# ChanghyeonKim93/nonlinear_optimizer_for_slam

Measured on AMD Instinct MI355X. Metric: ndt6_gauss_newton_residual_blocks_per_sec, higher is better.
Workload: dtype f64

## Files before the change

include/nos.h:

```cpp
#ifndef NOS_H_
#define NOS_H_

#include <stddef.h>
#include <stdint.h>

#ifdef __cplusplus
extern "C" {
#endif

#define NOS_NDT_PLANES 15
#define NOS_REPROJ_PLANES 5
#define NOS_NDT6_OUT 28
#define NOS_NDT3_OUT 10
#define NOS_REPROJ_OUT 28

typedef enum nos_status {
  NOS_OK = 0,
  NOS_ERR_INVALID_ARGUMENT = 1,
  NOS_ERR_NO_DEVICE = 2,
  NOS_ERR_HIP = 3,
  NOS_ERR_OUT_OF_MEMORY = 4,
  NOS_ERR_WRONG_KIND = 5,
  NOS_ERR_UNSUPPORTED = 6
} nos_status;
// ... 215 lines not shown
                            nos_register_report* reports);

int nos_voxel_map_register6_batch(nos_voxel_map* map, nos_scan* const* scans, int32_t n_problems, double* R, double* t,
                                  const nos_loss* loss, const nos_register_options* ropt, const nos_lm_options* options,
                                  nos_register_report* reports);
int nos_voxel_map_register3_batch(nos_voxel_map* map, nos_scan* const* scans, int32_t n_problems, double* R, double* t,
                                  const nos_loss* loss, const nos_register_options* ropt, const nos_lm_options* options,
                                  nos_register_report* reports);

typedef struct nos_pose_score {
  uint64_t matches;
  uint64_t matched_points;
  double cost;
  double reserved;
} nos_pose_score;

int nos_ndt_score_batch(nos_ndt_map* map, nos_scan* const* scans, int32_t n_problems, const double* R ,
                        const double* t , const nos_loss* loss, int max_neighbors, nos_pose_score* scores);
int nos_voxel_map_score_batch(nos_voxel_map* map, nos_scan* const* scans, int32_t n_problems, const double* R ,
                              const double* t , const nos_loss* loss, int max_neighbors, nos_pose_score* scores);

int nos_debug_lm_step(nos_ctx* ctx, int dof, const double* sums, const double settings[4], double state[22]);

int nos_debug_voxel_finish(uint32_t count, const double sums[9], const int64_t cell[3], double voxel_resolution,
                           const double params[3], int flags, double mean[3], double sqrt_information[9], unsigned char* valid);

int nos_debug_voxel_moments(uint32_t count, const double sums[9], const int64_t cell[3], double src_resolution,
                            const double R[9], const double t[3], double dst_resolution,
                            int64_t cell_out[3], double sums_out[9]);

typedef struct nos_pose_graph nos_pose_graph;
int nos_pgo_create(nos_ctx* ctx, size_t n_poses, const double* poses, size_t n_edges,
                   const int32_t* ref, const int32_t* qry, const double* meas,
                   const double* switch_init, const unsigned char* switch_free,
                   const unsigned char* fixed, nos_pose_graph** out_pg);
int nos_pgo_destroy(nos_pose_graph* pg);
size_t nos_pgo_num_unknowns(const nos_pose_graph* pg);
int nos_pgo_linearize(nos_pose_graph* pg, double* cost, double* gradient_norm);
int nos_pgo_solve(nos_pose_graph* pg, double lambda, int max_iterations, double rel_tolerance,
                  int* iterations, double* rel_residual, double* step_norm);
int nos_pgo_retract(nos_pose_graph* pg);
int nos_pgo_get_state(nos_pose_graph* pg, double* poses, double* switches);
int nos_pgo_get_vector(nos_pose_graph* pg, int which, double* out);
int nos_pgo_matvec(nos_pose_graph* pg, double lambda, const double* x, double* y);
int nos_pgo_layout_info(const nos_pose_graph* pg, unsigned long long info[8]);
int nos_pgo_time_sweep(nos_pose_graph* pg, int which, double lambda, int repeats, double* ms_per_sweep);
// ... 28 lines not shown
```

nonlinear_optimizer_for_slam_amd/_lib.py:

```python
import ctypes
import os

_HERE = os.path.dirname(os.path.abspath(__file__))
CSRC = os.path.join(_HERE, "csrc")
LIB_HIP = os.environ.get("NOS_HIP_LIB") or os.path.join(CSRC, "libnos_hip.so")
LIB_HOST = os.path.join(CSRC, "libnos_host.so")

c_double_p = ctypes.POINTER(ctypes.c_double)
c_void_pp = ctypes.POINTER(ctypes.c_void_p)

NOS_OK = 0
NOS_F64 = 0
NOS_F32 = 1
NOS_LOSS_NONE = 0
NOS_LOSS_EXPONENTIAL = 1
NOS_LOSS_HUBER = 2

C_ABI_SYMBOLS = (
    "nos_ctx_create", "nos_ctx_destroy", "nos_ctx_num_devices", "nos_ctx_set_stream",
    "nos_ctx_synchronize", "nos_comm_get_unique_id", "nos_ctx_comm_init", "nos_ctx_comm_size", "nos_ctx_comm_init_shm", "nos_ctx_comm_init_shm_device", "nos_comm_shm_unlink", "nos_ctx_comm_destroy",
    "nos_ctx_comm_allreduce", "nos_ndt_dataset_create", "nos_reproj_dataset_create",
    "nos_ndt_dataset_create_from_device", "nos_reproj_dataset_create_from_device",
    "nos_ndt_dataset_create_from_records", "nos_reproj_dataset_create_from_records",
    "nos_dataset_download", "nos_ndt_map_create", "nos_ndt_map_destroy", "nos_ndt_map_size", "nos_scan_create",
    "nos_scan_destroy", "nos_scan_size", "nos_scan_sort_by_cell", "nos_scan_order", "nos_scan_filter", "nos_scan_points", "nos_ndt_match", "nos_ndt_indexed_dataset_create", "nos_ndt_match_indexed", "nos_indexed_dataset_info", "nos_indexed_dataset_download", "nos_ndt_map_build", "nos_map_stats_size",
    "nos_map_stats_get", "nos_map_stats_get_eigen", "nos_map_stats_destroy",
    "nos_voxel_map_create", "nos_voxel_map_insert", "nos_voxel_map_insert_scan", "nos_voxel_map_info", "nos_voxel_map_snapshot",
    "nos_voxel_map_stats", "nos_voxel_map_match", "nos_voxel_map_match_indexed", "nos_voxel_map_prune", "nos_voxel_map_memory", "nos_voxel_map_merge", "nos_voxel_map_destroy", "nos_dataset_drop_last_matches", "nos_pgo_create", "nos_pgo_destroy", "nos_pgo_num_unknowns",
    "nos_pgo_linearize", "nos_pgo_solve", "nos_pgo_retract", "nos_pgo_get_state", "nos_pgo_get_vector",
    "nos_pgo_matvec", "nos_pgo_time_sweep", "nos_pgo_layout_info", "nos_debug_lm_step", "nos_debug_voxel_finish", "nos_debug_voxel_moments", "nos_dataset_destroy", "nos_dataset_size", "nos_dataset_dtype", "nos_dataset_stream_bytes",
    "nos_dataset_set_simd_class",
    "nos_ndt6_accumulate", "nos_ndt3_accumulate", "nos_reproj_accumulate",
    "nos_ndt6_accumulate_async", "nos_ndt3_accumulate_async", "nos_reproj_accumulate_async",
    "nos_ndt6_solve", "nos_ndt3_solve", "nos_reproj_solve",
    "nos_ndt6_solve_batch", "nos_ndt3_solve_batch", "nos_reproj_solve_batch",
    "nos_ndt6_register_batch", "nos_ndt3_register_batch", "nos_voxel_map_register6_batch", "nos_voxel_map_register3_batch",
    "nos_ndt_score_batch", "nos_voxel_map_score_batch",
    "nos_ctx_set_launch", "nos_ctx_set_option", "nos_ctx_get_option", "nos_runtime_info", "nos_ctx_comm_rccl_count",
    "nos_ctx_last_kernel", "nos_ctx_profile_begin", "nos_ctx_profile_end", "nos_ndt6_time_kernel", "nos_reproj_time_kernel",
    "nos_ndt3_time_kernel", "nos_status_string", "nos_last_error", "nos_version",
)


class NosLoss(ctypes.Structure):
    _fields_ = [("kind", ctypes.c_int32), ("reserved", ctypes.c_int32),
                ("a", ctypes.c_double), ("b", ctypes.c_double)]


class NosLmOptions(ctypes.Structure):
    _fields_ = [("max_iterations", ctypes.c_int32), ("launches_in_flight", ctypes.c_int32),
                ("gradient_tolerance", ctypes.c_double), ("parameter_tolerance", ctypes.c_double),
                ("cost_history", ctypes.POINTER(ctypes.c_double))]

# ... 132 lines not shown
        if hasattr(lib, "nos_voxel_map_match"):
            lib.nos_voxel_map_match.argtypes = [vp, vp, dp, dp, i, i, c_void_pp, ctypes.POINTER(sz)]
        if hasattr(lib, "nos_voxel_map_match_indexed"):
            lib.nos_voxel_map_match_indexed.argtypes = [vp, vp, dp, dp, i, i, i, c_void_pp, ctypes.POINTER(sz)]
            lib.nos_indexed_dataset_info.argtypes = [vp, ctypes.POINTER(i), ctypes.POINTER(sz)]
            lib.nos_indexed_dataset_download.argtypes = [vp, ctypes.POINTER(ctypes.POINTER(ctypes.c_int32)), dp]
    if hasattr(lib, "nos_dataset_drop_last_matches"):
        lib.nos_dataset_drop_last_matches.argtypes = [vp, sz]
    ip = ctypes.POINTER(ctypes.c_int32)
    lib.nos_pgo_create.argtypes = [vp, sz, dp, sz, ip, ip, dp, dp, ctypes.c_char_p, ctypes.c_char_p, c_void_pp]
    lib.nos_pgo_destroy.argtypes = [vp]
    lib.nos_pgo_num_unknowns.argtypes = [vp]
    lib.nos_pgo_num_unknowns.restype = sz
    lib.nos_pgo_linearize.argtypes = [vp, dp, dp]
    lib.nos_pgo_solve.argtypes = [vp, ctypes.c_double, i, ctypes.c_double, ctypes.POINTER(i), dp, dp]
    lib.nos_pgo_retract.argtypes = [vp]
    lib.nos_pgo_get_state.argtypes = [vp, dp, dp]
    lib.nos_pgo_get_vector.argtypes = [vp, i, dp]
    lib.nos_pgo_matvec.argtypes = [vp, ctypes.c_double, dp, dp]
    if hasattr(lib, "nos_pgo_layout_info"):
        lib.nos_pgo_layout_info.argtypes = [vp, ctypes.POINTER(ctypes.c_ulonglong)]
    if hasattr(lib, "nos_debug_lm_step"):
        lib.nos_debug_lm_step.argtypes = [vp, i, dp, dp, dp]
    if hasattr(lib, "nos_debug_voxel_finish"):
        lib.nos_debug_voxel_finish.argtypes = [ctypes.c_uint32, dp, ctypes.POINTER(ctypes.c_int64), ctypes.c_double, dp, i, dp, dp,
                                               ctypes.POINTER(ctypes.c_ubyte)]
    if hasattr(lib, "nos_debug_voxel_moments"):
        i64p = ctypes.POINTER(ctypes.c_int64)
        lib.nos_debug_voxel_moments.argtypes = [ctypes.c_uint32, dp, i64p, ctypes.c_double, dp, dp, ctypes.c_double, i64p, dp]
    if hasattr(lib, "nos_pgo_time_sweep"):
        lib.nos_pgo_time_sweep.argtypes = [vp, i, ctypes.c_double, i, dp]
    lib.nos_dataset_destroy.argtypes = [vp]
    lib.nos_dataset_set_simd_class.argtypes = [vp, ctypes.c_int]
    lib.nos_dataset_set_simd_class.restype = ctypes.c_int
    lib.nos_dataset_size.argtypes = [vp]
    lib.nos_dataset_size.restype = sz
    lib.nos_dataset_dtype.argtypes = [vp]
    lib.nos_dataset_stream_bytes.argtypes = [vp]
    lib.nos_dataset_stream_bytes.restype = sz
    lib.nos_ndt6_accumulate.argtypes = [vp, dp, dp, lp, dp]
    lib.nos_ndt3_accumulate.argtypes = [vp, dp, dp, lp, dp]
    lib.nos_reproj_accumulate.argtypes = [vp, dp, dp, dp, lp, ctypes.c_double, dp]
    lib.nos_ndt6_accumulate_async.argtypes = [vp, dp, dp, lp, vp]
    lib.nos_ndt3_accumulate_async.argtypes = [vp, dp, dp, lp, vp]
    lib.nos_reproj_accumulate_async.argtypes = [vp, dp, dp, dp, lp, ctypes.c_double, vp]
    lmo, lmr = ctypes.POINTER(NosLmOptions), ctypes.POINTER(NosLmReport)
# ... 33 lines not shown
```

nonlinear_optimizer_for_slam_amd/csrc/assemble_one_launch.hpp:

```cpp
#pragma once

#include "assemble_pass.hpp"

namespace nos {

constexpr size_t kSingleBlockMaxElements = size_t(1024) * 15;

template <typename Problem, typename T, int BLOCK, bool NT>
__device__ __forceinline__ int single_block_loop(const TiledLayout& L, typename Problem::Params& P, uint32_t n_chunks,
                                                 LmDevice& s_lm, double* s_sum, double* __restrict__ cost_history,
                                                 int history_capacity) {
  constexpr int kF = Problem::kFields;
  constexpr int kOut = Problem::kOut;
  const T* __restrict__ base = static_cast<const T*>(L.base);
  int executed = 0;
  while (s_lm.st.done == 0) {
    set_pose(P, &s_lm);
    T acc[kOut];
#pragma unroll
    for (int k = 0; k < kOut; ++k) acc[k] = T(0);
    constexpr uint32_t kRound = (kF * sizeof(T) > 64) ? 2 : 4;
    for (uint32_t c = 0; c < n_chunks; c += kRound) {
      T x[kRound][kF][1];
      uint64_t i0[kRound];
// ... 107 lines not shown
__device__ __forceinline__ void state_load_sc1(const LmDevice* lm, nos_host::LmState& st) {
  const double* d = reinterpret_cast<const double*>(&lm->st);
  double* s = reinterpret_cast<double*>(&st);
  constexpr int kWords = int(sizeof(nos_host::LmState) / sizeof(double));
#pragma unroll
  for (int k = 0; k < kWords; ++k) s[k] = sc1_load(d + k);
}

template <int FIELDS, int ELEM>
struct ResidentShape;
template <>
struct ResidentShape<15, 8> { static constexpr int RI = 3, LI = 3; };
template <>
struct ResidentShape<15, 4> { static constexpr int RI = 3, LI = 4; };
template <>
struct ResidentShape<5, 8> { static constexpr int RI = 9, LI = 7; };
template <>
struct ResidentShape<5, 4> { static constexpr int RI = 10, LI = 14; };

template <typename Problem, typename T>
struct StreamRegRounds { static constexpr int kRR = 3; };
template <int LOSS>
struct StreamRegRounds<Ndt6Problem<float, LOSS>, float> { static constexpr int kRR = 0; };
constexpr int kStreamRegRoundsMax = 3;

template <typename Problem, typename T, int BLOCK, int RI, int LI, int SI = 0, bool SPF = false, bool NT = false>
__global__ __launch_bounds__(BLOCK) void solve_cluster_kernel(TiledLayout L, typename Problem::Params P,
                                                             double* __restrict__ partials, LmDevice* lm, ClusterCtl* ctl,
                                                             double* __restrict__ cost_history, int history_capacity,
                                                             double* entry_host, unsigned long long* seq_host,
                                                             unsigned long long seq, uint32_t items_per_lane,
                                                             const Mailbox* mail = nullptr, uint32_t stream_lds = 0u,
                                                             uint32_t stream_reg = 0u) {
  constexpr int kF = Problem::kFields;
  constexpr int kOut = Problem::kOut;
  constexpr int kCols = 32;
  constexpr int kSlices = BLOCK / kCols;
  const T* __restrict__ base = static_cast<const T*>(L.base);
  constexpr int kRF = kF;
  extern __shared__ __align__(16) unsigned char resident_raw[];
  T* resident = reinterpret_cast<T*>(resident_raw);
  __shared__ int s_flag;
  __shared__ int s_fast;
  __shared__ double red[kSlices][kCols];
  __shared__ double s_tot[kLmTotDoubles(kOut)];
  __shared__ double s_lmd_raw[(sizeof(LmDevice) + 7) / 8];
  LmDevice& s_lmd = *reinterpret_cast<LmDevice*>(s_lmd_raw);
// ... 7 lines not shown
  [[maybe_unused]] constexpr int kXccCol = 28;
  [[maybe_unused]] const unsigned int my_xcc = xcc_id();
  const uint64_t block_base = uint64_t(blockIdx.x) * BLOCK * J;
  auto fetch = [&](uint32_t j, T (&dst)[kRF]) -> bool {
    const uint64_t i = block_base + uint64_t(j) * BLOCK + threadIdx.x;
    const bool ok = i < L.n;
    const uint64_t ic = ok ? i : 0;
    const uint64_t off = (ic >> L.tile_shift) * L.tile_stride + (ic & L.tile_mask);
    T xt[kF][1];
#pragma unroll
    for (int f = 0; f < kF; ++f) load_items<T, 1, false>(base + field_offset<Problem>(L, ic, off, f), xt[f]);
#pragma unroll
    for (int f = 0; f < kF; ++f) dst[f] = ok ? xt[f][0] : T(0);
    return ok;
  };
  auto evaluate_resident = [&](const T (&xi)[kRF], bool ok, T (&acc_)[kOut]) { Problem::item(xi, P, ok, acc_); };
  T x[RI > 0 ? RI : 1][kRF];
  bool valid[RI > 0 ? RI : 1];
  static_assert(SI == 0 || (RI == 0 && LI == 0), "the streaming form keeps nothing resident");
  constexpr int kSI = SI > 0 ? SI : 1;
  [[maybe_unused]] T xs[kF][kSI];
  [[maybe_unused]] uint64_t xs_i0 = 0;
  [[maybe_unused]] constexpr int kRR = (SI > 0 && !SPF) ? StreamRegRounds<Problem, T>::kRR : 0;
  static_assert(kRR <= kStreamRegRoundsMax, "the option's range covers every instantiation");
  [[maybe_unused]] T xr[kRR > 0 ? kRR : 1][kF][kSI];
  [[maybe_unused]] const uint32_t my_rounds = blockIdx.x < J ? (J - blockIdx.x + gridDim.x - 1) / gridDim.x : 0u;
  [[maybe_unused]] const uint32_t lds_k = SI > 0 ? min(stream_lds, my_rounds > 0u ? my_rounds - 1u : 0u) : 0u;
  [[maybe_unused]] const uint32_t reg_k = kRR > 0 ? min(min(stream_reg, uint32_t(kRR)), (my_rounds > 0u ? my_rounds - 1u : 0u) - lds_k) : 0u;
  [[maybe_unused]] const uint32_t alt_k = min(lds_k, reg_k);
  [[maybe_unused]] auto chip_round = [&](uint32_t i) -> uint32_t {
    return uint32_t(uint64_t(i + 1u) * my_rounds / (lds_k + reg_k + 1u));
  };
  [[maybe_unused]] auto lds_slot_round = [&](uint32_t sl) -> uint32_t {
    return sl < lds_k ? chip_round(sl < alt_k ? 2u * sl : alt_k + sl) : ~0u;
  };
  [[maybe_unused]] const uint32_t lds_r0 = lds_slot_round(0u);
  [[maybe_unused]] const uint32_t lds_r1 = lds_slot_round(1u);
  [[maybe_unused]] const uint32_t lds_r2 = lds_slot_round(2u);
  [[maybe_unused]] uint32_t reg_r[kRR > 0 ? kRR : 1];
#pragma unroll
  for (int j = 0; j < (kRR > 0 ? kRR : 1); ++j)
    reg_r[j] = uint32_t(j) < reg_k ? chip_round(uint32_t(j) < alt_k ? 2u * uint32_t(j) + 1u : alt_k + uint32_t(j)) : ~0u;
#pragma unroll
  for (int j = 0; j < (kRR > 0 ? kRR : 1); ++j)
#pragma unroll
    for (int f = 0; f < kF; ++f)
#pragma unroll
      for (int e = 0; e < kSI; ++e) xr[j][f][e] = T(0);
  [[maybe_unused]] auto lds_round = [&](uint32_t s) -> uint32_t { return s == 0u ? lds_r0 : s == 1u ? lds_r1 : s == 2u ? lds_r2 : ~0u; };
  [[maybe_unused]] auto fetch_chunk = [&](uint32_t c, T (&dst)[kF][kSI]) -> uint64_t {
    const uint64_t i0 = uint64_t(c) * (uint64_t(BLOCK) * kSI) + uint64_t(threadIdx.x) * kSI;
    const uint64_t off = (i0 >> L.tile_shift) * L.tile_stride + (i0 & L.tile_mask);
#pragma unroll
    for (int f = 0; f < kF; ++f) load_items<T, kSI, NT>(base + field_offset<Problem>(L, i0, off, f), dst[f]);
    return i0;
  };
  if constexpr (SI > 0) {
    if (blockIdx.x < J) xs_i0 = fetch_chunk(blockIdx.x, xs);
  }
#pragma unroll
  for (int j = 0; j < RI; ++j) {
    valid[j] = false;
    if (uint32_t(j) < J) {
      valid[j] = fetch(uint32_t(j), x[j]);
    } else {
#pragma unroll
      for (int f = 0; f < kRF; ++f) x[j][f] = T(0);
    }
  }
  if constexpr (LI > 0) {
    for (uint32_t j = RI; j < J; ++j) {
      T xi[kRF];
      (void)fetch(j, xi);
#pragma unroll
      for (int f = 0; f < kRF; ++f) resident[(size_t(j - RI) * kRF + f) * BLOCK + threadIdx.x] = xi[f];
    }
  }
// ... 159 lines not shown
      }
    } else
    if (sizeof(T) == 8 && J >= uint32_t(RI)) {
#pragma unroll
      for (int j = 0; j < RI; ++j) evaluate_resident(x[j], valid[j], acc);
    } else {
#pragma unroll
      for (int j = 0; j < RI; ++j)
        if (uint32_t(j) < J) evaluate_resident(x[j], valid[j], acc);
    }
    if constexpr (LI > 0) {
      for (uint32_t j = RI; j < J; ++j) {
        T xi[kRF];
#pragma unroll
        for (int f = 0; f < kRF; ++f) xi[f] = resident[(size_t(j - RI) * kRF + f) * BLOCK + threadIdx.x];
        evaluate_resident(xi, (block_base + uint64_t(j) * BLOCK + threadIdx.x) < L.n, acc);
      }
    }
    double dacc[kOut];
#pragma unroll
    for (int k = 0; k < kOut; ++k) dacc[k] = double(acc[k]);
    NOS_RES_STAMP(0)
    {
      TaggedUnit* const block_units = reinterpret_cast<TaggedUnit*>(partials);
      TaggedUnit* const group_units = block_units + size_t(kClusterMaxBlocks) * 32;
      const unsigned long long tag = (seq << 24) | ((unsigned long long)it + 1ull);
      const double mine = block_reduce_value<kOut, BLOCK>(dacc);
      const bool probe = it == 0u && allow_fast;
      if (threadIdx.x < kOut) {
        if (s_fast != 0)
          tagged_store_plain(block_units + size_t(blockIdx.x) * 32 + threadIdx.x, mine, tag);
        else
          tagged_store(block_units + size_t(blockIdx.x) * 32 + threadIdx.x, mine, tag);
      } else if (probe && threadIdx.x == kXccCol) {
        tagged_store(block_units + size_t(blockIdx.x) * 32 + kXccCol, double(my_xcc), tag);
      }
      NOS_RES_STAMP(1)
      const unsigned long long deadline = wall_clock64() + (multi ? kClusterMailboxTimeoutTicks : kClusterTimeoutTicks);
      auto await = [&](const TaggedUnit* u, double* value) -> bool {
        unsigned int polls = 0;
        for (;;) {
          const TaggedUnit got = tagged_load(u);
          if (got.seq == tag) {
            *value = got.value;
            return true;
          }
          if ((++polls & 63u) == 0u &&
              (__hip_atomic_load(&ctl->abort, __ATOMIC_RELAXED, __HIP_MEMORY_SCOPE_AGENT) != 0u || wall_clock64() > deadline)) {
            __hip_atomic_store(&ctl->abort, 1u, __ATOMIC_RELAXED, __HIP_MEMORY_SCOPE_AGENT);
            s_flag = 2;
            return false;
          }
        }
      };
      const int col = threadIdx.x % kCols;
      const int slice = threadIdx.x / kCols;
      if (blockIdx.x < n_groups) {
        const unsigned int g_size = (gridDim.x - blockIdx.x + 7u) >> 3;
        double gsum = 0.0;
        for (unsigned int m0 = 0; m0 < g_size; m0 += kSlices) {
          const unsigned int m = m0 + slice;
          double v = 0.0;
          if (m < g_size && (col < kOut || (probe && col == kXccCol))) {
            (void)await(block_units + size_t(blockIdx.x + 8u * m) * 32 + col, &v);
            if (col == kXccCol) v = v == double(my_xcc) ? 0.0 : 1.0;
          }
          red[slice][col] = v;
          __syncthreads();
          if (threadIdx.x < kOut || (probe && threadIdx.x == kXccCol)) {
#pragma unroll
            for (int sl = 0; sl < kSlices; ++sl) gsum += red[sl][threadIdx.x];
          }
          __syncthreads();
        }
        if ((threadIdx.x < kOut || (probe && threadIdx.x == kXccCol)) && s_flag != 2)
          tagged_store(group_units + (size_t(it & 1u) * 8 + blockIdx.x) * 32 + threadIdx.x, gsum, tag);
      }
      if (!multi || blockIdx.x == 0) {
        double v = 0.0;
        if (slice < int(n_groups) && (col < kOut || (probe && col == kXccCol)) && s_flag != 2)
          (void)await(group_units + (size_t(it & 1u) * 8 + slice) * 32 + col, &v);
        if (slice < 8) red[slice][col] = v;
      }
      __syncthreads();
      if (multi) {
        TaggedUnit* const global_units = group_units + size_t(2) * 8 * 32;
        if (blockIdx.x == 0) {
          if (threadIdx.x < kCols && s_flag != 2) {
            double tot = 0.0;
            if (threadIdx.x < kOut || (probe && threadIdx.x == kXccCol))
              for (unsigned int g = 0; g < n_groups; ++g) tot += red[g][threadIdx.x];
            s_local[threadIdx.x] = tot;
          }
          __syncthreads();
          if (threadIdx.x < kWave) {
            const Mailbox mb = *mail;
            const unsigned long long round = s_round0 + (unsigned long long)it + 1ull;
            const unsigned int xtag = (unsigned int)(round % 0xFFFFFFFFull) + 1u;
            const size_t parity = size_t(round & 1ull);
            const size_t units_base = size_t(mb.n_ranks) * 2 * kMailSlotDoubles;
            const int lane = int(threadIdx.x);
            const bool giving_up = s_flag == 2;
            unsigned long long* const own = reinterpret_cast<unsigned long long*>(mb.peers[mb.rank] + units_base);
            if (giving_up) {
              if (lane < mb.n_ranks)
                __hip_atomic_store(reinterpret_cast<unsigned long long*>(mb.peers[lane] + units_base) +
                                       (size_t(mb.rank) * 2 + parity) * kMailSlotDoubles + 63,
                                   (unsigned long long)xtag << 32, __ATOMIC_RELAXED, __HIP_MEMORY_SCOPE_SYSTEM);
            } else {
              unsigned long long gran = 0ull;
              if (lane < 2 * kOut) {
                const unsigned long long bits = (unsigned long long)__double_as_longlong(s_local[lane >> 1]);
                gran = ((unsigned long long)xtag << 32) | ((lane & 1) ? (bits >> 32) : (bits & 0xFFFFFFFFull));
                for (int p = 0; p < mb.n_ranks; ++p)
                  __hip_atomic_store(reinterpret_cast<unsigned long long*>(mb.peers[p] + units_base) +
                                         (size_t(mb.rank) * 2 + parity) * kMailSlotDoubles + lane,
                                     gran, __ATOMIC_RELAXED, __HIP_MEMORY_SCOPE_SYSTEM);
              }
              double sum = 0.0;
              bool lost = false;
              const unsigned long long give_up_at = wall_clock64() + kClusterMailboxTimeoutTicks;
              for (int r = 0; r < mb.n_ranks && !lost; ++r) {
                const unsigned long long* slot_r = own + (size_t(r) * 2 + parity) * kMailSlotDoubles;
                unsigned long long got = 0ull;
// ... 15 lines not shown
                }
                const unsigned int half = (unsigned int)(got & 0xFFFFFFFFull);
                const unsigned int other = (unsigned int)__shfl_xor(int(half), 1, kWave);
                const double value = __longlong_as_double((long long)(((unsigned long long)((lane & 1) ? half : other) << 32) |
                                                                      (unsigned long long)((lane & 1) ? other : half)));
                sum += value;
              }
              if (lost) {
                if (lane == 0) {
                  __hip_atomic_store(&ctl->abort, 1u, __ATOMIC_RELAXED, __HIP_MEMORY_SCOPE_AGENT);
                  s_flag = 2;
                }
                if (lane < mb.n_ranks)
                  __hip_atomic_store(reinterpret_cast<unsigned long long*>(mb.peers[lane] + units_base) +
                                         (size_t(mb.rank) * 2 + parity) * kMailSlotDoubles + 63,
                                     (unsigned long long)xtag << 32, __ATOMIC_RELAXED, __HIP_MEMORY_SCOPE_SYSTEM);
              } else if (lane < 2 * kOut && (lane & 1) == 0) {
                s_local[lane >> 1] = sum;
              }
            }
          }
          __syncthreads();
          if (s_flag != 2) {
            if (threadIdx.x < kOut || (probe && threadIdx.x == kXccCol))
              tagged_store(global_units + size_t(it & 1u) * 32 + threadIdx.x, s_local[threadIdx.x], tag);
          }
        }
        {
          double v = 0.0;
          if (threadIdx.x < kCols && (col < kOut || (probe && col == kXccCol)) && s_flag != 2)
            (void)await(global_units + size_t(it & 1u) * 32 + col, &v);
          if (threadIdx.x < kCols) red[0][col] = v;
        }
        __syncthreads();
      }
      NOS_RES_STAMP(2)
      if (s_flag == 2) break;
      if (multi) {
        if (threadIdx.x < kOut)
          s_tot[threadIdx.x] = red[0][threadIdx.x];
        else if (probe && threadIdx.x == kXccCol)
          s_fast = red[0][kXccCol] == 0.0 ? 1 : 0;
      } else
      if (threadIdx.x < kOut) {
        double tot = 0.0;
        for (unsigned int g = 0; g < n_groups; ++g) tot += red[g][threadIdx.x];
        s_tot[threadIdx.x] = tot;
      } else if (probe && threadIdx.x == kXccCol) {
        double strangers = 0.0;
        for (unsigned int g = 0; g < n_groups; ++g) strangers += red[g][kXccCol];
        s_fast = strangers == 0.0 ? 1 : 0;
      }
      __syncthreads();
    }
    {
      NOS_RES_STAMP(3)
      if (threadIdx.x == 0) {
        if (blockIdx.x == 0 && cost_history != nullptr && executed < history_capacity)
          __hip_atomic_store(cost_history + executed, s_tot[kOut - 1], __ATOMIC_RELAXED, __HIP_MEMORY_SCOPE_SYSTEM);
        lm_step_lane<kOut>(lds_ptr(s_tot), lds_ptr(&s_lmd));
        s_flag = s_state.done != 0 ? 1 : 0;
      }
    }
    ++executed;
    ++it;
    __syncthreads();
    NOS_RES_STAMP(4)
  }
  NOS_PROBE(
  if (blockIdx.x == 0 && threadIdx.x == 0 && entry_host != nullptr) {
    for (int k = 0; k < 5; ++k)
// ... 43 lines not shown
```

nonlinear_optimizer_for_slam_amd/csrc/nos_core.hip:

```cpp
#include "nos_internal.hpp"

namespace nosd {


thread_local const void* t_last_kernel = nullptr;

template <typename Problem, typename T, int ITEMS, int BLOCK, int MINW, int PREFETCH = 0>
int launch_variant(const nos::TiledLayout& L, const typename Problem::Params& P, int grid_cap, int num_cus_hint,
                   bool nt, double* partials, const nos::FusedFinal& fin_in, hipStream_t stream, int* rows_out) {
  constexpr uint32_t kChunk = BLOCK * ITEMS;
  if (L.n_padded % kChunk != 0) return fail(NOS_ERR_INVALID_ARGUMENT, "n_padded %% chunk != 0");
  if (L.tile_stride != 0 && ((size_t(L.tile_mask) + 1) % kChunk) != 0)
    return fail(NOS_ERR_INVALID_ARGUMENT, "tile not a multiple of the kernel chunk");
  const uint64_t n_chunks64 = L.n_padded / kChunk;
  if (n_chunks64 > 0xFFFFFFFFull) return fail(NOS_ERR_UNSUPPORTED, "dataset too large for one shard");
  const uint32_t n_chunks = uint32_t(n_chunks64);
  int grid = int(std::min<uint64_t>(n_chunks, uint64_t(grid_cap)));
  if (grid < 1) grid = 1;
  if (grid > kMaxPartialRows) grid = kMaxPartialRows;
  nos::FusedFinal fin = fin_in;
  fin.write_through = (fin.counter != nullptr && grid <= num_cus_hint && fin_in.write_through != 0) ? 1 : 0;
  const auto kernel = nt ? nos::assemble_kernel<Problem, T, ITEMS, BLOCK, MINW, true, PREFETCH>
                         : nos::assemble_kernel<Problem, T, ITEMS, BLOCK, MINW, false, PREFETCH>;
  t_last_kernel = reinterpret_cast<const void*>(kernel);
// ... 55 lines not shown
#undef NOS_CASE
#undef NOS_CASE_PP
  return fail(NOS_ERR_UNSUPPORTED, "launch geometry %d is not compiled into this build for this element type "
              "(default build: fp64 0, 1, 3, 7; fp32 1, 11; `make ALL_VARIANTS=1` builds the rest)", variant);
}

size_t resident_items_per_lane(int n_fields, int dtype) {
  if (n_fields == 15)
    return dtype == NOS_F64 ? size_t(nos::ResidentShape<15, 8>::RI + nos::ResidentShape<15, 8>::LI)
                            : size_t(nos::ResidentShape<15, 4>::RI + nos::ResidentShape<15, 4>::LI);
  if (n_fields == 5)
    return dtype == NOS_F64 ? size_t(nos::ResidentShape<5, 8>::RI + nos::ResidentShape<5, 8>::LI)
                            : size_t(nos::ResidentShape<5, 4>::RI + nos::ResidentShape<5, 4>::LI);
  return 1;
}

struct SingleBlockArgs {
  int cluster_blocks = 0;
  int items_per_lane = 1;
  int stream_chunks = 0;
  bool nt = false;
  int stream_lds_chunks = 0;
  int stream_reg_rounds = 0;
  bool stage1_sc1 = false;
  const nos::Mailbox* mail = nullptr;
  double* partials = nullptr;
  nos::ClusterCtl* ctl = nullptr;
  nos::LmDevice* lm;
  double* history;
  int history_capacity;
  double* entry;
  unsigned long long* seq_host;
  unsigned long long seq;
};

template <typename Problem, typename T>
int launch_single(const nos::TiledLayout& L, const typename Problem::Params& P, const SingleBlockArgs& a, hipStream_t stream) {
  constexpr int kBlock = 512;
  if (L.n_padded % kBlock != 0) return fail(NOS_ERR_INVALID_ARGUMENT, "n_padded %% 512 != 0");
  if (a.cluster_blocks > 0 && a.stream_chunks > 0) {
    constexpr int kSI = sizeof(T) == 8 ? 1 : 2;
    constexpr bool kSPF = false;
    constexpr size_t kChunk = size_t(kBlock) * kSI;
    if (L.n_padded % kChunk != 0 || (L.tile_stride != 0 && ((size_t(L.tile_mask) + 1) % kChunk) != 0))
      return fail(NOS_ERR_INVALID_ARGUMENT, "streaming solve: layout not a multiple of the %zu-item chunk", kChunk);
    if (size_t(a.stream_chunks) * kChunk != L.n_padded) return fail(NOS_ERR_INVALID_ARGUMENT, "streaming solve: chunk count does not match the layout");
    const auto kernel = a.nt ? nos::solve_cluster_kernel<Problem, T, kBlock, 0, 0, kSI, kSPF, true>
                             : nos::solve_cluster_kernel<Problem, T, kBlock, 0, 0, kSI, kSPF, false>;
    uint32_t lds = uint32_t(std::min(std::max(a.stream_lds_chunks, 0), 3));
    size_t dyn_bytes = lds * size_t(Problem::kFields) * kChunk * sizeof(T);
    if (dyn_bytes > size_t(48) * 1024 &&
        hipFuncSetAttribute(reinterpret_cast<const void*>(kernel), hipFuncAttributeMaxDynamicSharedMemorySize,
                            int(dyn_bytes)) != hipSuccess) {
      (void)hipGetLastError();
      lds = 0;
      dyn_bytes = 0;
    }
    const uint32_t reg = uint32_t(std::min(std::max(a.stream_reg_rounds, 0), nos::kStreamRegRoundsMax));
    t_last_kernel = reinterpret_cast<const void*>(kernel);
    hipLaunchKernelGGL(kernel, dim3(a.cluster_blocks), dim3(kBlock), dyn_bytes, stream, L, P, a.partials, a.lm, a.ctl, a.history,
                       a.history_capacity, a.entry, a.seq_host, a.seq, uint32_t(a.stream_chunks) | (a.stage1_sc1 ? 0x80000000u : 0u),
                       a.mail, lds, reg);
    hipError_t e = hipGetLastError();
    if (e != hipSuccess) return fail(NOS_ERR_HIP, "streaming solve launch failed: %s", hipGetErrorString(e));
    return NOS_OK;
  }
  if (a.cluster_blocks > 0) {
    using Shape = nos::ResidentShape<Problem::kPlanes, int(sizeof(T))>;
    if (a.items_per_lane < 1 || a.items_per_lane > Shape::RI + Shape::LI)
      return fail(NOS_ERR_INVALID_ARGUMENT, "resident solve: %d items per lane do not fit (%d + %d)", a.items_per_lane,
                  Shape::RI, Shape::LI);
    const auto kernel = nos::solve_cluster_kernel<Problem, T, kBlock, Shape::RI, Shape::LI>;
    const size_t lds_items = a.items_per_lane > Shape::RI ? size_t(a.items_per_lane - Shape::RI) : 0;
    const size_t dyn_bytes = lds_items * size_t(Problem::kFields) * kBlock * sizeof(T);
    if (dyn_bytes > size_t(48) * 1024) {
      const hipError_t ea = hipFuncSetAttribute(reinterpret_cast<const void*>(kernel),
                                                hipFuncAttributeMaxDynamicSharedMemorySize, int(dyn_bytes));
      if (ea != hipSuccess) return fail(NOS_ERR_UNSUPPORTED, "resident solve: %zu bytes of LDS refused: %s", dyn_bytes, hipGetErrorString(ea));
    }
    t_last_kernel = reinterpret_cast<const void*>(kernel);
    hipLaunchKernelGGL(kernel, dim3(a.cluster_blocks), dim3(kBlock), dyn_bytes, stream, L, P, a.partials, a.lm, a.ctl,
// ... 401 lines not shown
  const bool stream_form = !resident_fits && (ctx->settings.lm_cluster == 1 || ctx->settings.lm_cluster == 5) && items_per_lane >= 1 &&
                           sh.layout.n_padded % stream_chunk == 0 && sh.layout.n_padded / stream_chunk < (size_t(1) << 31) &&
                           (sh.layout.tile_stride == 0 || (size_t(sh.layout.tile_mask) + 1) % stream_chunk == 0);
  bool paused = false;
  if (mailbox_in_launch) {
    paused = slot.cluster_paused_solves > 0;
    if (paused) --slot.cluster_paused_solves;
  } else {
    if (slot.cluster_gave_up &&
        std::chrono::steady_clock::now() - slot.cluster_gave_up_at > std::chrono::milliseconds(ctx->settings.lm_cluster_retry_ms))
      slot.cluster_gave_up = false;
    paused = slot.cluster_gave_up;
  }
  if (!cluster_eligible(ds, opt, mailbox_in_launch, cluster_blocks, resident_fits, stream_form, paused)) return NOS_OK;
  SingleBlockArgs cl{};
  cl.cluster_blocks = int(cluster_blocks);
  cl.items_per_lane = int(items_per_lane);
  if (stream_form) {
    cl.items_per_lane = 0;
    cl.stream_chunks = int(sh.layout.n_padded / stream_chunk);
    cl.nt = use_nontemporal(ds, sh);
    cl.stream_lds_chunks = ctx->settings.stream_lds_chunks;
    cl.stream_reg_rounds = ctx->settings.stream_reg_rounds;
  }
  cl.stage1_sc1 = ctx->settings.lm_cluster == 5;
  cl.mail = mailbox_in_launch ? ctx->d_mail : nullptr;
  cl.partials = slot.partials;
  cl.ctl = slot.d_cluster;
  cl.lm = slot.d_lm;
  cl.history = opt->cost_history ? slot.h_hist_dev : nullptr;
  cl.history_capacity = kHistCapacity;
  cl.entry = slot.h_log_dev;
  cl.seq_host = reinterpret_cast<unsigned long long*>(slot.h_out_dev + kSeqSlot);
  cl.seq = ++slot.seq;
  NOS_HIP_CHECK(hipMemsetAsync(slot.d_cluster, 0, sizeof(nos::ClusterCtl), slot.stream));
  if (ctx->settings.debug_cluster_abort != 0) {
    const unsigned int raised = 1u;
    NOS_HIP_CHECK(hipMemcpyAsync(&slot.d_cluster->abort, &raised, sizeof raised, hipMemcpyHostToDevice, slot.stream));
    NOS_HIP_CHECK(hipStreamSynchronize(slot.stream));
  }
  int rows = 0;
  const int rc_launch = launch_assemble_raw(ds, sh, rq, slot.partials, nos::FusedFinal{}, slot.stream, &rows, &cl);
  if (rc_launch != NOS_OK && rc_launch != NOS_ERR_UNSUPPORTED) return rc_launch;
  const bool launched_ok = rc_launch == NOS_OK;
  *finished = launched_ok && spin_for_sequence(slot, cl.seq, 4000000);
  if (!*finished) {
// ... 212 lines not shown
  return with_request(2, ds, R, 9, t, 3, intr, min_depth, loss,
                      [&](const Request& rq) { return lm_solve(ds, rq, options, R, 9, t, 3, report); });
}

int nos_ndt6_time_kernel(nos_dataset* ds, const double R[9], const double t[3], const nos_loss* loss, int repeats,
                         double* kernel_ms, double* total_ms) {
  return with_request(6, ds, R, 9, t, 3, nullptr, 0.0, loss,
                      [&](const Request& rq) { return time_kernel(ds, rq, repeats, kernel_ms, total_ms); });
}

int nos_ndt3_time_kernel(nos_dataset* ds, const double R2[4], const double t2[2], const nos_loss* loss, int repeats,
                         double* kernel_ms, double* total_ms) {
  return with_request(3, ds, R2, 4, t2, 2, nullptr, 0.0, loss,
                      [&](const Request& rq) { return time_kernel(ds, rq, repeats, kernel_ms, total_ms); });
}

int nos_reproj_time_kernel(nos_dataset* ds, const double R[9], const double t[3], const double intr[4],
                           const nos_loss* loss, double min_depth, int repeats, double* kernel_ms,
                           double* total_ms) {
  return with_request(2, ds, R, 9, t, 3, intr, min_depth, loss,
                      [&](const Request& rq) { return time_kernel(ds, rq, repeats, kernel_ms, total_ms); });
}

int nos_debug_lm_step(nos_ctx* ctx, int dof, const double* sums, const double settings[4], double state[22]) {
  nosd::CtxGuard guard_(ctx);
  if (!ctx || !sums || !settings || !state || (dof != 6 && dof != 3)) return fail(NOS_ERR_INVALID_ARGUMENT, "bad argument");
  DeviceSlot& slot = ctx->slots[0];
  NOS_HIP_CHECK(hipSetDevice(slot.device));
  nos::LmDevice lmd{};
  for (int k = 0; k < 9; ++k) lmd.st.R[k] = state[k];
  for (int k = 0; k < 3; ++k) lmd.st.t[k] = state[9 + k];
  lmd.st.q.w = state[12], lmd.st.q.x = state[13], lmd.st.q.y = state[14], lmd.st.q.z = state[15];
  lmd.st.lambda = state[16], lmd.st.previous_cost = state[17], lmd.st.cost = state[18];
  lmd.st.iteration = int(state[19]), lmd.st.done = int(state[20]), lmd.st.ok = int(state[21]);
  lmd.settings.max_iterations = int(settings[0]);
  lmd.settings.gradient_tolerance = settings[1];
  lmd.settings.parameter_tolerance = settings[2];
  lmd.settings.float_schedule = int(settings[3]);
  const int n_out = dof == 6 ? 28 : 10;
  NOS_HIP_CHECK(hipMemcpyAsync(slot.d_lm, &lmd, sizeof lmd, hipMemcpyHostToDevice, slot.stream));
  NOS_HIP_CHECK(hipMemcpyAsync(slot.d_out, sums, sizeof(double) * n_out, hipMemcpyHostToDevice, slot.stream));
  NOS_HIP_CHECK(hipStreamSynchronize(slot.stream));
  if (dof == 6)
    hipLaunchKernelGGL((nos::lm_step_kernel<28>), dim3(1), dim3(64), 0, slot.stream, slot.d_out, slot.d_lm,
                       static_cast<double*>(nullptr), static_cast<unsigned long long*>(nullptr), 0ull);
  else
// ... 15 lines not shown
```

nonlinear_optimizer_for_slam_amd/csrc/nos_ctx.hip:

```cpp
#include "nos_internal.hpp"

#include <cxxabi.h>

namespace nosd {

namespace {
thread_local std::string g_last_error;
}

int fail(int status, const char* fmt, ...) {
  char buf[512];
  va_list ap;
  va_start(ap, fmt);
  vsnprintf(buf, sizeof buf, fmt, ap);
  va_end(ap);
  g_last_error = buf;
  return status;
}

const char* last_error_text() { return g_last_error.c_str(); }
void clear_last_error() { g_last_error.clear(); }

std::string dir_of_symbol(const void* symbol, std::string* file_out) {
  Dl_info info{};
// ... 80 lines not shown
    {"lm_fused", &nosd::Settings::lm_fused, 0, 1},
    {"lm_window", &nosd::Settings::lm_window, 1, nosd::kLogSlots - 2},
    {"lm_single", &nosd::Settings::lm_single, 0, 1},
    {"lm_cluster", &nosd::Settings::lm_cluster, 0, 5},
    {"lm_cluster_retry_ms", &nosd::Settings::lm_cluster_retry_ms, 0, 3600000},
    {"pool", &nosd::Settings::pool, 0, 1},
    {"tile_log2", &nosd::Settings::tile_log2, -1, 24},
    {"ingest", &nosd::Settings::ingest, 0, 2},
    {"ingest_threads", &nosd::Settings::ingest_threads, 0, 1024},
    {"indexed_bpc", &nosd::Settings::indexed_bpc, 1, 16},
    {"match_dense", &nosd::Settings::match_dense, 0, 1},
    {"map_compact_keys", &nosd::Settings::map_compact_keys, 0, 1},
    {"pgo_host_scalars", &nosd::Settings::pgo_host_scalars, 0, 1},
    {"pgo_precond", &nosd::Settings::pgo_precond, 0, 1},
    {"pgo_agg", &nosd::Settings::pgo_agg, 2, 1 << 20},
    {"pgo_block", &nosd::Settings::pgo_block, 0, 1},
    {"pgo_coarse_probe", &nosd::Settings::pgo_coarse_probe, 0, 1},
    {"map_fma_mask", &nosd::Settings::map_fma_mask, 0, (1 << 26) - 1},
    {"map_eigen_version", &nosd::Settings::map_eigen_version, 33, 34},
    {"debug_cluster_abort", &nosd::Settings::debug_cluster_abort, 0, 2},
    {"lm_cluster_max_blocks", &nosd::Settings::lm_cluster_max_blocks, 1, 256},
    {"stream_lds_chunks", &nosd::Settings::stream_lds_chunks, 0, 3},
    {"stream_reg_rounds", &nosd::Settings::stream_reg_rounds, 0, nos::kStreamRegRoundsMax},
    {"batch_max_elements", &nosd::Settings::batch_max_elements, 0, 1 << 30},
};
bool option_in_range(const OptionEntry& o, int value) {
  if (value < o.lo || value > o.hi) return false;
  if (!strcmp(o.key, "tile_log2")) return value <= 0 || value >= 10;
  return true;
}
void drop_out_of_range_settings(nosd::Settings& st) {
  const nosd::Settings defaults;
  for (const OptionEntry& o : kOptions)
    if (!option_in_range(o, st.*(o.field))) {
      fprintf(stderr, "[nos-hip] NOS_%s = %d is outside [%d, %d]: ignored\n", o.key, st.*(o.field), o.lo, o.hi);
      st.*(o.field) = defaults.*(o.field);
    }
}
}


extern "C" {

int nos_ctx_create(const int* device_ids, int n_devices, nos_ctx** out_ctx) {
  if (!out_ctx) return fail(NOS_ERR_INVALID_ARGUMENT, "out_ctx is NULL");
  *out_ctx = nullptr;
// ... 4 lines not shown
    return fail(NOS_ERR_NO_DEVICE, "no usable HIP device (%s); this library has no CPU fallback",
                e != hipSuccess ? hipGetErrorString(e) : "device count is 0");
  for (int i = 0; i < n_devices; ++i)
    if (device_ids[i] < 0 || device_ids[i] >= count)
      return fail(NOS_ERR_INVALID_ARGUMENT, "device id %d out of range [0,%d)", device_ids[i], count);
  nos_ctx* ctx = new (std::nothrow) nos_ctx();
  if (!ctx) return fail(NOS_ERR_OUT_OF_MEMORY, "host allocation failed");
  ctx->slots.resize(n_devices);
  ctx->blocks_per_cu = env_int("NOS_BLOCKS_PER_CU", 0);
  ctx->variant = env_int("NOS_VARIANT", 0);
  {
    Settings& st = ctx->settings;
    st.plane_skew = env_int("NOS_PLANE_SKEW", st.plane_skew);
    st.sc1 = env_int("NOS_SC1", st.sc1);
    st.nt = env_int("NOS_NT", st.nt);
    st.fused = env_int("NOS_FUSED", st.fused);
    st.lm_fused = env_int("NOS_LM_FUSED", st.lm_fused);
    st.lm_window = env_int("NOS_LM_WINDOW", st.lm_window);
    st.lm_single = env_int("NOS_LM_SINGLE", st.lm_single);
    st.lm_cluster = env_int("NOS_LM_CLUSTER", st.lm_cluster);
    st.lm_cluster_max_blocks = env_int("NOS_LM_CLUSTER_MAX_BLOCKS", st.lm_cluster_max_blocks);
    st.stream_lds_chunks = env_int("NOS_STREAM_LDS_CHUNKS", st.stream_lds_chunks);
    st.stream_reg_rounds = env_int("NOS_STREAM_REG_ROUNDS", st.stream_reg_rounds);
    st.batch_max_elements = env_int("NOS_BATCH_MAX_ELEMENTS", st.batch_max_elements);
    st.pool = env_int("NOS_POOL", st.pool);
    st.tile_log2 = env_int("NOS_TILE_LOG2", st.tile_log2);
    const char* ingest = getenv("NOS_INGEST");
    st.ingest = (ingest && !strcmp(ingest, "pack")) ? 1 : ((ingest && !strcmp(ingest, "unpack")) ? 2 : 0);
    st.ingest_threads = env_int("NOS_INGEST_THREADS", 0);
    st.indexed_bpc = env_int("NOS_INDEXED_BPC", st.indexed_bpc);
    st.match_dense = env_int("NOS_MATCH_DENSE", st.match_dense);
    st.map_compact_keys = env_int("NOS_MAP_COMPACT_KEYS", st.map_compact_keys);
    st.pgo_host_scalars = env_int("NOS_PGO_HOST_SCALARS", st.pgo_host_scalars);
    st.pgo_precond = env_int("NOS_PGO_PRECOND", st.pgo_precond);
    st.pgo_agg = env_int("NOS_PGO_AGG", st.pgo_agg);
    st.pgo_block = env_int("NOS_PGO_BLOCK", st.pgo_block);
    st.pgo_coarse_probe = env_int("NOS_PGO_COARSE_PROBE", st.pgo_coarse_probe);
    drop_out_of_range_settings(st);
  }
  for (int i = 0; i < n_devices; ++i) {
    DeviceSlot& s = ctx->slots[i];
    s.device = device_ids[i];
    s.pool_enabled = ctx->settings.pool != 0;
    hipDeviceProp_t prop;
    e = hipSetDevice(s.device);
    if (e == hipSuccess) e = hipGetDeviceProperties(&prop, s.device);
// ... 262 lines not shown
```

nonlinear_optimizer_for_slam_amd/csrc/nos_internal.hpp:

```cpp
#pragma once

#include <hip/hip_runtime.h>
#include <dlfcn.h>
#include <fcntl.h>
#include <sys/mman.h>
#include <sys/stat.h>
#include <unistd.h>
#include <rccl/rccl.h>

#include <algorithm>
#include <atomic>
#include <chrono>
#include <random>
#include <climits>
#include <cmath>
#include <cstdarg>
#include <cstdio>
#include <cstdlib>
#include <cstring>
#include <map>
#include <memory>
#include <new>
#include <string>
#include <thread>
// ... 116 lines not shown
  int lm_fused = 1;
  int lm_window = 3;
  int lm_single = 1;
  int lm_cluster_retry_ms = 5000;
  int lm_cluster = 1;
  int pool = 1;
  int tile_log2 = -1;
  int ingest = 0;
  int ingest_threads = 0;
  int indexed_bpc = 1;
  int match_dense = 1;
  int map_compact_keys = 1;
  int pgo_host_scalars = 0;
  int pgo_precond = 1;
  int pgo_agg = 48;
  int pgo_coarse_probe = 0;
  int pgo_block = 1;
  int map_fma_mask = kMapReferenceFmaMask;
  int map_eigen_version = 34;
  int debug_cluster_abort = 0;
  int lm_cluster_max_blocks = 256;
  int stream_lds_chunks = 3;
  int stream_reg_rounds = 3;
  int batch_max_elements = int(nos::kSingleBlockMaxElements);
};
}

struct nos_ctx {
  std::recursive_mutex mu;
  nosd::Settings settings;
  std::vector<nosd::DeviceSlot> slots;
  int blocks_per_cu = 0;
  int variant = 0;
  int tile_log2 = -1;
  ncclComm_t comm = nullptr;
  int comm_ranks = 1;
  int comm_rank = 0;
  void* shm_host = nullptr;
  size_t shm_bytes = 0;
  double* shm_dev = nullptr;
  unsigned long long* d_round = nullptr;
  nos::Mailbox* d_mail = nullptr;
  double* ipc_own = nullptr;
  std::vector<double*> ipc_peers;
  double** d_peers = nullptr;
};
// ... 279 lines not shown
```

Measured before the change: 77.10 billion.

## Deepen register streaming rounds for f64 NDT problems with tight pointer-stepped loads

Raises the number of register-held prefetch rounds for the f64 NDT6 kernel (3 or 4 depending on loss) and for NDT3 (5), controlled by a new stream_reg_extra setting that defaults to the maximum. When the deeper streaming is active, field loads use a single global pointer advanced by the field stride, with asm barriers to keep address arithmetic cheap. threadIdx.x is also pinned in a register for the reduction code. The intent is to hide more memory latency per block, at the cost of higher register pressure and possible occupancy loss or spills.

Measured after the change: 77.07 billion. About the same (-0.0%).

```diff
diff --git a/include/nos.h b/include/nos.h
--- a/include/nos.h
+++ b/include/nos.h
@@ -261,6 +261,8 @@
 
 int nos_debug_lm_step(nos_ctx* ctx, int dof, const double* sums, const double settings[4], double state[22]);
 
+int nos_debug_stream_reg_slots(int problem, int dtype, int loss_kind);
+
 int nos_debug_voxel_finish(uint32_t count, const double sums[9], const int64_t cell[3], double voxel_resolution,
                            const double params[3], int flags, double mean[3], double sqrt_information[9], unsigned char* valid);
 
diff --git a/nonlinear_optimizer_for_slam_amd/_lib.py b/nonlinear_optimizer_for_slam_amd/_lib.py
--- a/nonlinear_optimizer_for_slam_amd/_lib.py
+++ b/nonlinear_optimizer_for_slam_amd/_lib.py
@@ -28,7 +28,7 @@
     "nos_voxel_map_create", "nos_voxel_map_insert", "nos_voxel_map_insert_scan", "nos_voxel_map_info", "nos_voxel_map_snapshot",
     "nos_voxel_map_stats", "nos_voxel_map_match", "nos_voxel_map_match_indexed", "nos_voxel_map_prune", "nos_voxel_map_memory", "nos_voxel_map_merge", "nos_voxel_map_destroy", "nos_dataset_drop_last_matches", "nos_pgo_create", "nos_pgo_destroy", "nos_pgo_num_unknowns",
     "nos_pgo_linearize", "nos_pgo_solve", "nos_pgo_retract", "nos_pgo_get_state", "nos_pgo_get_vector",
-    "nos_pgo_matvec", "nos_pgo_time_sweep", "nos_pgo_layout_info", "nos_debug_lm_step", "nos_debug_voxel_finish", "nos_debug_voxel_moments", "nos_dataset_destroy", "nos_dataset_size", "nos_dataset_dtype", "nos_dataset_stream_bytes",
+    "nos_pgo_matvec", "nos_pgo_time_sweep", "nos_pgo_layout_info", "nos_debug_lm_step", "nos_debug_stream_reg_slots", "nos_debug_voxel_finish", "nos_debug_voxel_moments", "nos_dataset_destroy", "nos_dataset_size", "nos_dataset_dtype", "nos_dataset_stream_bytes",
     "nos_dataset_set_simd_class",
     "nos_ndt6_accumulate", "nos_ndt3_accumulate", "nos_reproj_accumulate",
     "nos_ndt6_accumulate_async", "nos_ndt3_accumulate_async", "nos_reproj_accumulate_async",
@@ -207,6 +207,8 @@
         lib.nos_pgo_layout_info.argtypes = [vp, ctypes.POINTER(ctypes.c_ulonglong)]
     if hasattr(lib, "nos_debug_lm_step"):
         lib.nos_debug_lm_step.argtypes = [vp, i, dp, dp, dp]
+    if hasattr(lib, "nos_debug_stream_reg_slots"):
+        lib.nos_debug_stream_reg_slots.argtypes = [i, i, i]
     if hasattr(lib, "nos_debug_voxel_finish"):
         lib.nos_debug_voxel_finish.argtypes = [ctypes.c_uint32, dp, ctypes.POINTER(ctypes.c_int64), ctypes.c_double, dp, i, dp, dp,
                                                ctypes.POINTER(ctypes.c_ubyte)]
diff --git a/nonlinear_optimizer_for_slam_amd/csrc/assemble_one_launch.hpp b/nonlinear_optimizer_for_slam_amd/csrc/assemble_one_launch.hpp
--- a/nonlinear_optimizer_for_slam_amd/csrc/assemble_one_launch.hpp
+++ b/nonlinear_optimizer_for_slam_amd/csrc/assemble_one_launch.hpp
@@ -153,7 +153,12 @@
 struct StreamRegRounds { static constexpr int kRR = 3; };
 template <int LOSS>
 struct StreamRegRounds<Ndt6Problem<float, LOSS>, float> { static constexpr int kRR = 0; };
+template <int LOSS>
+struct StreamRegRounds<Ndt6Problem<double, LOSS>, double> { static constexpr int kRR = LOSS == kLossExponential ? 3 : 4; };
+template <int LOSS>
+struct StreamRegRounds<Ndt3Problem<double, LOSS>, double> { static constexpr int kRR = 5; };
 constexpr int kStreamRegRoundsMax = 3;
+constexpr int kStreamRegExtraMax = 2;
 
 template <typename Problem, typename T, int BLOCK, int RI, int LI, int SI = 0, bool SPF = false, bool NT = false>
 __global__ __launch_bounds__(BLOCK) void solve_cluster_kernel(TiledLayout L, typename Problem::Params P,
@@ -207,7 +212,8 @@
   [[maybe_unused]] T xs[kF][kSI];
   [[maybe_unused]] uint64_t xs_i0 = 0;
   [[maybe_unused]] constexpr int kRR = (SI > 0 && !SPF) ? StreamRegRounds<Problem, T>::kRR : 0;
-  static_assert(kRR <= kStreamRegRoundsMax, "the option's range covers every instantiation");
+  static_assert(kRR <= kStreamRegRoundsMax + kStreamRegExtraMax, "the two options' ranges cover every instantiation");
+  [[maybe_unused]] constexpr bool kStreamTight = kRR > kStreamRegRoundsMax;
   [[maybe_unused]] T xr[kRR > 0 ? kRR : 1][kF][kSI];
   [[maybe_unused]] const uint32_t my_rounds = blockIdx.x < J ? (J - blockIdx.x + gridDim.x - 1) / gridDim.x : 0u;
   [[maybe_unused]] const uint32_t lds_k = SI > 0 ? min(stream_lds, my_rounds > 0u ? my_rounds - 1u : 0u) : 0u;
@@ -236,8 +242,31 @@
   [[maybe_unused]] auto fetch_chunk = [&](uint32_t c, T (&dst)[kF][kSI]) -> uint64_t {
     const uint64_t i0 = uint64_t(c) * (uint64_t(BLOCK) * kSI) + uint64_t(threadIdx.x) * kSI;
     const uint64_t off = (i0 >> L.tile_shift) * L.tile_stride + (i0 & L.tile_mask);
-#pragma unroll
-    for (int f = 0; f < kF; ++f) load_items<T, kSI, NT>(base + field_offset<Problem>(L, i0, off, f), dst[f]);
+    if constexpr (!Problem::kSPlanes && kStreamTight) {
+      using V = typename VecOf<T, kSI>::type;
+      typedef const V __attribute__((address_space(1)))* GlobalPtr;
+      uint64_t a = reinterpret_cast<uint64_t>(base + off);
+      const uint64_t step = L.field_stride * sizeof(T);
+#pragma unroll
+      for (int f = 0; f < kF; ++f) {
+        V v;
+        if constexpr (NT)
+          v = __builtin_nontemporal_load((GlobalPtr)a);
+        else
+          v = *(GlobalPtr)a;
+        if constexpr (kSI == 1) {
+          dst[f][0] = v;
+        } else {
+#pragma unroll
+          for (int k = 0; k < kSI; ++k) dst[f][k] = v[k];
+        }
+        a += step;
+        asm("" : "+v"(a));
+      }
+    } else {
+#pragma unroll
+      for (int f = 0; f < kF; ++f) load_items<T, kSI, NT>(base + field_offset<Problem>(L, i0, off, f), dst[f]);
+    }
     return i0;
   };
   if constexpr (SI > 0) {
@@ -443,17 +472,19 @@
     for (int k = 0; k < kOut; ++k) dacc[k] = double(acc[k]);
     NOS_RES_STAMP(0)
     {
+      unsigned int tx = threadIdx.x;
+      if constexpr (kStreamTight) asm volatile("" : "+v"(tx));
       TaggedUnit* const block_units = reinterpret_cast<TaggedUnit*>(partials);
       TaggedUnit* const group_units = block_units + size_t(kClusterMaxBlocks) * 32;
       const unsigned long long tag = (seq << 24) | ((unsigned long long)it + 1ull);
       const double mine = block_reduce_value<kOut, BLOCK>(dacc);
       const bool probe = it == 0u && allow_fast;
-      if (threadIdx.x < kOut) {
+      if (tx < kOut) {
         if (s_fast != 0)
-          tagged_store_plain(block_units + size_t(blockIdx.x) * 32 + threadIdx.x, mine, tag);
+          tagged_store_plain(block_units + size_t(blockIdx.x) * 32 + tx, mine, tag);
         else
-          tagged_store(block_units + size_t(blockIdx.x) * 32 + threadIdx.x, mine, tag);
-      } else if (probe && threadIdx.x == kXccCol) {
+          tagged_store(block_units + size_t(blockIdx.x) * 32 + tx, mine, tag);
+      } else if (probe && tx == kXccCol) {
         tagged_store(block_units + size_t(blockIdx.x) * 32 + kXccCol, double(my_xcc), tag);
       }
       NOS_RES_STAMP(1)
@@ -474,8 +505,8 @@
           }
         }
       };
-      const int col = threadIdx.x % kCols;
-      const int slice = threadIdx.x / kCols;
+      const int col = tx % kCols;
+      const int slice = tx / kCols;
       if (blockIdx.x < n_groups) {
         const unsigned int g_size = (gridDim.x - blockIdx.x + 7u) >> 3;
         double gsum = 0.0;
@@ -488,14 +519,14 @@
           }
           red[slice][col] = v;
           __syncthreads();
-          if (threadIdx.x < kOut || (probe && threadIdx.x == kXccCol)) {
-#pragma unroll
-            for (int sl = 0; sl < kSlices; ++sl) gsum += red[sl][threadIdx.x];
+          if (tx < kOut || (probe && tx == kXccCol)) {
+#pragma unroll
+            for (int sl = 0; sl < kSlices; ++sl) gsum += red[sl][tx];
           }
           __syncthreads();
         }
-        if ((threadIdx.x < kOut || (probe && threadIdx.x == kXccCol)) && s_flag != 2)
-          tagged_store(group_units + (size_t(it & 1u) * 8 + blockIdx.x) * 32 + threadIdx.x, gsum, tag);
+        if ((tx < kOut || (probe && tx == kXccCol)) && s_flag != 2)
+          tagged_store(group_units + (size_t(it & 1u) * 8 + blockIdx.x) * 32 + tx, gsum, tag);
       }
       if (!multi || blockIdx.x == 0) {
         double v = 0.0;
@@ -507,20 +538,20 @@
       if (multi) {
         TaggedUnit* const global_units = group_units + size_t(2) * 8 * 32;
         if (blockIdx.x == 0) {
-          if (threadIdx.x < kCols && s_flag != 2) {
+          if (tx < kCols && s_flag != 2) {
             double tot = 0.0;
-            if (threadIdx.x < kOut || (probe && threadIdx.x == kXccCol))
-              for (unsigned int g = 0; g < n_groups; ++g) tot += red[g][threadIdx.x];
-            s_local[threadIdx.x] = tot;
+            if (tx < kOut || (probe && tx == kXccCol))
+              for (unsigned int g = 0; g < n_groups; ++g) tot += red[g][tx];
+            s_local[tx] = tot;
           }
           __syncthreads();
-          if (threadIdx.x < kWave) {
+          if (tx < kWave) {
             const Mailbox mb = *mail;
             const unsigned long long round = s_round0 + (unsigned long long)it + 1ull;
             const unsigned int xtag = (unsigned int)(round % 0xFFFFFFFFull) + 1u;
             const size_t parity = size_t(round & 1ull);
             const size_t units_base = size_t(mb.n_ranks) * 2 * kMailSlotDoubles;
-            const int lane = int(threadIdx.x);
+            const int lane = int(tx);
             const bool giving_up = s_flag == 2;
             unsigned long long* const own = reinterpret_cast<unsigned long long*>(mb.peers[mb.rank] + units_base);
             if (giving_up) {
@@ -582,31 +613,31 @@
           }
           __syncthreads();
           if (s_flag != 2) {
-            if (threadIdx.x < kOut || (probe && threadIdx.x == kXccCol))
-              tagged_store(global_units + size_t(it & 1u) * 32 + threadIdx.x, s_local[threadIdx.x], tag);
+            if (tx < kOut || (probe && tx == kXccCol))
+              tagged_store(global_units + size_t(it & 1u) * 32 + tx, s_local[tx], tag);
           }
         }
         {
           double v = 0.0;
-          if (threadIdx.x < kCols && (col < kOut || (probe && col == kXccCol)) && s_flag != 2)
+          if (tx < kCols && (col < kOut || (probe && col == kXccCol)) && s_flag != 2)
             (void)await(global_units + size_t(it & 1u) * 32 + col, &v);
-          if (threadIdx.x < kCols) red[0][col] = v;
+          if (tx < kCols) red[0][col] = v;
         }
         __syncthreads();
       }
       NOS_RES_STAMP(2)
       if (s_flag == 2) break;
       if (multi) {
-        if (threadIdx.x < kOut)
-          s_tot[threadIdx.x] = red[0][threadIdx.x];
-        else if (probe && threadIdx.x == kXccCol)
+        if (tx < kOut)
+          s_tot[tx] = red[0][tx];
+        else if (probe && tx == kXccCol)
           s_fast = red[0][kXccCol] == 0.0 ? 1 : 0;
       } else
-      if (threadIdx.x < kOut) {
+      if (tx < kOut) {
         double tot = 0.0;
-        for (unsigned int g = 0; g < n_groups; ++g) tot += red[g][threadIdx.x];
-        s_tot[threadIdx.x] = tot;
-      } else if (probe && threadIdx.x == kXccCol) {
+        for (unsigned int g = 0; g < n_groups; ++g) tot += red[g][tx];
+        s_tot[tx] = tot;
+      } else if (probe && tx == kXccCol) {
         double strangers = 0.0;
         for (unsigned int g = 0; g < n_groups; ++g) strangers += red[g][kXccCol];
         s_fast = strangers == 0.0 ? 1 : 0;
diff --git a/nonlinear_optimizer_for_slam_amd/csrc/nos_core.hip b/nonlinear_optimizer_for_slam_amd/csrc/nos_core.hip
--- a/nonlinear_optimizer_for_slam_amd/csrc/nos_core.hip
+++ b/nonlinear_optimizer_for_slam_amd/csrc/nos_core.hip
@@ -101,6 +101,7 @@
   bool nt = false;
   int stream_lds_chunks = 0;
   int stream_reg_rounds = 0;
+  int stream_reg_extra = 0;
   bool stage1_sc1 = false;
   const nos::Mailbox* mail = nullptr;
   double* partials = nullptr;
@@ -135,7 +136,8 @@
       lds = 0;
       dyn_bytes = 0;
     }
-    const uint32_t reg = uint32_t(std::min(std::max(a.stream_reg_rounds, 0), nos::kStreamRegRoundsMax));
+    uint32_t reg = uint32_t(std::min(std::max(a.stream_reg_rounds, 0), nos::kStreamRegRoundsMax));
+    if (reg == uint32_t(nos::kStreamRegRoundsMax)) reg += uint32_t(std::min(std::max(a.stream_reg_extra, 0), nos::kStreamRegExtraMax));
     t_last_kernel = reinterpret_cast<const void*>(kernel);
     hipLaunchKernelGGL(kernel, dim3(a.cluster_blocks), dim3(kBlock), dyn_bytes, stream, L, P, a.partials, a.lm, a.ctl, a.history,
                        a.history_capacity, a.entry, a.seq_host, a.seq, uint32_t(a.stream_chunks) | (a.stage1_sc1 ? 0x80000000u : 0u),
@@ -583,6 +585,7 @@
     cl.nt = use_nontemporal(ds, sh);
     cl.stream_lds_chunks = ctx->settings.stream_lds_chunks;
     cl.stream_reg_rounds = ctx->settings.stream_reg_rounds;
+    cl.stream_reg_extra = ctx->settings.stream_reg_extra;
   }
   cl.stage1_sc1 = ctx->settings.lm_cluster == 5;
   cl.mail = mailbox_in_launch ? ctx->d_mail : nullptr;
@@ -841,6 +844,24 @@
                       [&](const Request& rq) { return time_kernel(ds, rq, repeats, kernel_ms, total_ms); });
 }
 
+int nos_debug_stream_reg_slots(int problem, int dtype, int loss_kind) {
+  if ((dtype != NOS_F64 && dtype != NOS_F32) || loss_kind < NOS_LOSS_NONE || loss_kind > NOS_LOSS_HUBER) return -1;
+  if (problem == 0) return nos::kStreamRegRoundsMax + nos::kStreamRegExtraMax;
+  return with_loss(loss_kind, [&](auto loss) -> int {
+    constexpr int kLoss = decltype(loss)::value;
+    const bool f64 = dtype == NOS_F64;
+    switch (problem) {
+      case 6: return f64 ? nos::StreamRegRounds<nos::Ndt6Problem<double, kLoss>, double>::kRR
+                         : nos::StreamRegRounds<nos::Ndt6Problem<float, kLoss>, float>::kRR;
+      case 3: return f64 ? nos::StreamRegRounds<nos::Ndt3Problem<double, kLoss>, double>::kRR
+                         : nos::StreamRegRounds<nos::Ndt3Problem<float, kLoss>, float>::kRR;
+      case 2: return f64 ? nos::StreamRegRounds<nos::ReprojProblem<double, kLoss>, double>::kRR
+                         : nos::StreamRegRounds<nos::ReprojProblem<float, kLoss>, float>::kRR;
+      default: return -1;
+    }
+  });
+}
+
 int nos_debug_lm_step(nos_ctx* ctx, int dof, const double* sums, const double settings[4], double state[22]) {
   nosd::CtxGuard guard_(ctx);
   if (!ctx || !sums || !settings || !state || (dof != 6 && dof != 3)) return fail(NOS_ERR_INVALID_ARGUMENT, "bad argument");
diff --git a/nonlinear_optimizer_for_slam_amd/csrc/nos_ctx.hip b/nonlinear_optimizer_for_slam_amd/csrc/nos_ctx.hip
--- a/nonlinear_optimizer_for_slam_amd/csrc/nos_ctx.hip
+++ b/nonlinear_optimizer_for_slam_amd/csrc/nos_ctx.hip
@@ -126,6 +126,7 @@
     {"lm_cluster_max_blocks", &nosd::Settings::lm_cluster_max_blocks, 1, 256},
     {"stream_lds_chunks", &nosd::Settings::stream_lds_chunks, 0, 3},
     {"stream_reg_rounds", &nosd::Settings::stream_reg_rounds, 0, nos::kStreamRegRoundsMax},
+    {"stream_reg_extra", &nosd::Settings::stream_reg_extra, 0, nos::kStreamRegExtraMax},
     {"batch_max_elements", &nosd::Settings::batch_max_elements, 0, 1 << 30},
 };
 bool option_in_range(const OptionEntry& o, int value) {
@@ -176,6 +177,7 @@
     st.lm_cluster_max_blocks = env_int("NOS_LM_CLUSTER_MAX_BLOCKS", st.lm_cluster_max_blocks);
     st.stream_lds_chunks = env_int("NOS_STREAM_LDS_CHUNKS", st.stream_lds_chunks);
     st.stream_reg_rounds = env_int("NOS_STREAM_REG_ROUNDS", st.stream_reg_rounds);
+    st.stream_reg_extra = env_int("NOS_STREAM_REG_EXTRA", st.stream_reg_extra);
     st.batch_max_elements = env_int("NOS_BATCH_MAX_ELEMENTS", st.batch_max_elements);
     st.pool = env_int("NOS_POOL", st.pool);
     st.tile_log2 = env_int("NOS_TILE_LOG2", st.tile_log2);
diff --git a/nonlinear_optimizer_for_slam_amd/csrc/nos_internal.hpp b/nonlinear_optimizer_for_slam_amd/csrc/nos_internal.hpp
--- a/nonlinear_optimizer_for_slam_amd/csrc/nos_internal.hpp
+++ b/nonlinear_optimizer_for_slam_amd/csrc/nos_internal.hpp
@@ -162,6 +162,7 @@
   int lm_cluster_max_blocks = 256;
   int stream_lds_chunks = 3;
   int stream_reg_rounds = 3;
+  int stream_reg_extra = nos::kStreamRegExtraMax;
   int batch_max_elements = int(nos::kSingleBlockMaxElements);
 };
 }
```
